# pmgbergen/porepy

Measured on NVIDIA H100. Metric: 3D cells/sec MPFA+MPSA assembly, higher is better.
Workload: dtype f64

## Files before the change

porepy_b200/csrc/mpsa_node.cuh:

```cuda
#pragma once
#include "node_kernels.cuh"

namespace pb {

PB_HD int mpsa_width(int nd, int nsf, int nsc, int nb, int nalpha) {
    return (nsf * nd + nsc * nd + nb * nd + nalpha * nsc) | 1;
}
PB_HD int64_t mpsa_A_doubles(int nd, int nsf, int nsc, int nb, int nalpha) {
    return (int64_t)nsf * nd * mpsa_width(nd, nsf, nsc, nb, nalpha);
}
PB_HD int64_t mpsa_rest_doubles(int nd, int nsf, int nsc, int nb, int nalpha) {
    const int64_t nd2 = nd * nd, n = (int64_t)nsf * nd;
    const int64_t nrhs = (int64_t)nsc * nd + (int64_t)nb * nd + (int64_t)nalpha * nsc;
    int64_t d = (int64_t)nsc * nd2 * nd2;
    d += (int64_t)nsc * nd2;
    d += nd2 * (n + (int64_t)nsc * nd);
    d += nd2 * nrhs;
    d += nsf;
    d += (int64_t)nsf * nd;
    d += (int64_t)nsc;
    d += (int64_t)nalpha * nsc * nd2 * 2;
    int64_t ints = nsc + 4 * (int64_t)nsf + (int64_t)nsf * nd + n + (int64_t)nsc * nd + 2 * nd;
    return d + (ints + 1) / 2 + 2;
}
// ... 96 lines not shown
        for (int q = 0; q < nal; ++q) {
            const double *al = prm.alpha + (int64_t)q * prm.alpha_stride;
            double a2[ND][ND];
#pragma unroll
            for (int a = 0; a < ND; ++a)
#pragma unroll
                for (int b = 0; b < ND; ++b) a2[a][b] = al[(3 * a + b) * prm.alpha_cs + c * prm.alpha_es];
#pragma unroll
            for (int m = 0; m < ND; ++m) {
                const int u = slot[k * ND + m] >> 1;
#pragma unroll
                for (int i = 0; i < ND; ++i) {
                    double v = 0.0, w = 0.0;
#pragma unroll
                    for (int r = 0; r < ND; ++r) {
                        v += nrm[u * ND + r] * a2[r][i];
                        w += a2[i][r] * Ei[r][m];
                    }
                    NA[((q * nsc + k) * ND + m) * ND + i] = v;
                    AE[((q * nsc + k) * ND + i) * ND + m] = w;
                }
            }
        }
    }
    t.sync();
    for (int it = t.tid(); it < nsc * ND2; it += t.size()) {
        const int k = it / ND2, p = it - k * ND2;
        const int64_t c = cell[k];
        const int pi = p / ND, pr = p - pi * ND;
        const double *Crow = prm.stiff + (int64_t)c9<ND>(pi, pr) * 9 * prm.stiff_cs + c * prm.stiff_es;
#pragma unroll
        for (int a = 0; a < ND; ++a) {
            double cs[ND];
#pragma unroll
            for (int q = 0; q < ND; ++q)
                cs[q] = sym_mask<ND>(p, a * ND + q) ? Crow[(int64_t)c9<ND>(a, q) * prm.stiff_cs] : 0.0;
#pragma unroll
            for (int m = 0; m < ND; ++m) {
                double v = 0.0;
#pragma unroll
                for (int q = 0; q < ND; ++q) v += cs[q] * E[k * ND2 + q * ND + m];
                PS[((k * ND2 + p) * ND + a) * ND + m] = v;
            }
        }
    }
    for (int it = t.tid(); it < ND2 * ND * nsc; it += t.size()) {
        const int pa = it / nsc, k = it - pa * nsc;
        const int p = pa / ND, a = pa - p * ND;
        const int pi = p / ND, pr = p - pi * ND;
        double tot = 0.0;
        for (int j = 0; j < nsc; ++j) tot += volk[j];
        const double w = volk[k] / tot;
        const int64_t c = cell[k];
        const double *Crow = prm.stiff + (int64_t)c9<ND>(pi, pr) * 9 * prm.stiff_cs + c * prm.stiff_es;
        double ca[ND];
#pragma unroll
        for (int q = 0; q < ND; ++q)
            ca[q] = sym_mask<ND>(p, a * ND + q) ? 0.0 : w * Crow[(int64_t)c9<ND>(a, q) * prm.stiff_cs];
        double sum = 0.0;
#pragma unroll
        for (int m = 0; m < ND; ++m) {
            double v = 0.0;
#pragma unroll
            for (int q = 0; q < ND; ++q) v += ca[q] * E[k * ND2 + q * ND + m];
            team_add(SA + p * n + (slot[k * ND + m] >> 1) * ND + a, v);
            sum += v;
        }
        SAc[p * ncc + k * ND + a] = -sum;
    }
    for (int i = t.tid(); i < ND; i += t.size()) {
        int cn = 0, cr = 0;
        for (int u = 0; u < nsf; ++u) {
            cn += bcu[u * ND + i] == 2;
            cr += bcu[u * ND + i] == 3;
        }
        elim[i] = nsc < cn;
        elim[ND + i] = nsc < cr;
    }
    t.sync();

    for (int u = t.tid(); u < nsf; u += t.size()) {
        const int s1 = sides[u] & 0xFFFF, s2 = (sides[u] >> 16) & 0xFFFF;
        int pick = s1;
        if (s2 != 0xFFFF) {
            const double *nu = nrm + u * ND;
            double w1 = 0.0, w2 = 0.0;
            const double *p1 = PS + (s1 / ND) * ND2 * ND2, *p2 = PS + (s2 / ND) * ND2 * ND2;
            for (int i = 0; i < ND; ++i)
                for (int am = 0; am < ND2; ++am) {
                    double a1 = 0.0, a2 = 0.0;
#pragma unroll
                    for (int r = 0; r < ND; ++r) {
                        a1 += nu[r] * p1[(i * ND + r) * ND2 + am];
                        a2 += nu[r] * p2[(i * ND + r) * ND2 + am];
                    }
                    w1 += fabs(a1);
                    w2 += fabs(a2);
                }
            if (w2 < w1) pick = s2;
        }
        sidesel[u] = pick;
    }
    t.sync();

    auto row_of = [&](int x, double *row) {
        const int u = x / ND, i = x - u * ND;
        const int code = bcu[x];
        if (code == 1 && prm.basis == nullptr) {
            row[x] = 1.0;
            row[n + ncc + bloc[u] * ND + i] = 1.0;
            return;
        }
        const double *nu = nrm + u * ND;
        if (prm.basis != nullptr && bloc[u] >= 0) {
            const int64_t fb = face[u];
            double B[ND][ND];
#pragma unroll
            for (int a = 0; a < ND; ++a)
#pragma unroll
                for (int j = 0; j < ND; ++j) B[a][j] = prm.basis[(int64_t)(a * ND + j) * nf + fb];
            if (code == 1) {
#pragma unroll
                for (int j = 0; j < ND; ++j) row[u * ND + j] = B[i][j];
                row[n + ncc + bloc[u] * ND + i] = 1.0;
            } else {
                const int side = sides[u] & 0xFFFF;
                const int k = side / ND;
                const double sg = (slot[side] & 1) ? -1.0 : 1.0;
                for (int j = 0; j < ND; ++j) {
                    const double wgt = sg * B[i][j];
                    if (wgt == 0.0) continue;
                    const double *ps = PS + (k * ND2 + j * ND) * ND2;
#pragma unroll
                    for (int a = 0; a < ND; ++a) {
                        double csum = 0.0;
#pragma unroll
                        for (int m = 0; m < ND; ++m) {
                            double v = 0.0;
#pragma unroll
                            for (int r = 0; r < ND; ++r) v += nu[r] * ps[(r * ND + a) * ND + m];
                            v *= wgt;
                            row[(slot[k * ND + m] >> 1) * ND + a] += v;
                            csum += v;
                        }
                        row[n + k * ND + a] += csum;
                    }
                    for (int q = 0; q < nal; ++q)
                        row[n + ncc + nbc + q * nsc + k] += wgt * NA[((q * nsc + k) * ND + (side - k * ND)) * ND + j];
                    const int cj = bcu[u * ND + j];
                    if (!((cj == 2 && elim[j]) || (cj == 3 && elim[ND + j]))) {
                        for (int c = 0; c < n; ++c) {
                            double v = 0.0;
#pragma unroll
                            for (int r = 0; r < ND; ++r) v += nu[r] * SA[(j * ND + r) * n + c];
                            row[c] += wgt * v;
                        }
                        for (int c = 0; c < ncc; ++c) {
                            double v = 0.0;
#pragma unroll
                            for (int r = 0; r < ND; ++r) v += nu[r] * SAc[(j * ND + r) * ncc + c];
                            row[n + c] -= wgt * v;
                        }
                    }
                }
                row[n + ncc + bloc[u] * ND + i] = invmf[u];
                if (code == 3) {
                    const double as = G.farea[fb] * invmf[u];
#pragma unroll
                    for (int j = 0; j < ND; ++j) {
                        double wb = 0.0;
#pragma unroll
                        for (int kk = 0; kk < ND; ++kk)
                            wb += (prm.robw ? prm.robw[(int64_t)(i * ND + kk) * nf + fb] : (i == kk ? 1.0 : 0.0)) * B[kk][j];
                        row[u * ND + j] += as * wb;
                    }
                }
            }
            return;
        }
        for (int sd = 0; sd < 2; ++sd) {
            const int side = sd == 0 ? (sides[u] & 0xFFFF) : ((sides[u] >> 16) & 0xFFFF);
            if (side == 0xFFFF) continue;
            const int k = side / ND;
            const double sg = (slot[side] & 1) ? -1.0 : 1.0;
            const double *ps = PS + (k * ND2 + i * ND) * ND2;
#pragma unroll
            for (int a = 0; a < ND; ++a) {
                double csum = 0.0;
#pragma unroll
                for (int m = 0; m < ND; ++m) {
                    double v = 0.0;
#pragma unroll
                    for (int r = 0; r < ND; ++r) v += nu[r] * ps[(r * ND + a) * ND + m];
                    v *= sg;
                    row[(slot[k * ND + m] >> 1) * ND + a] += v;
                    csum += v;
                }
                row[n + k * ND + a] += csum;
            }
            for (int q = 0; q < nal; ++q)
                row[n + ncc + nbc + q * nsc + k] += sg * NA[((q * nsc + k) * ND + (side - k * ND)) * ND + i];
            if (code != 0) {
                const bool el = code == 2 ? elim[i] : elim[ND + i];
                if (!el) {
                    for (int c = 0; c < n; ++c) {
                        double v = 0.0;
#pragma unroll
                        for (int r = 0; r < ND; ++r) v += nu[r] * SA[(i * ND + r) * n + c];
                        row[c] += sg * v;
                    }
                    for (int c = 0; c < ncc; ++c) {
                        double v = 0.0;
#pragma unroll
                        for (int r = 0; r < ND; ++r) v += nu[r] * SAc[(i * ND + r) * ncc + c];
                        row[n + c] -= sg * v;
                    }
                }
            }
        }
        if (code == 2 || code == 3) row[n + ncc + bloc[u] * ND + i] = invmf[u];
        if (code == 3) {
            const int64_t f = face[u];
            const double as = G.farea[f] * invmf[u];
#pragma unroll
            for (int j = 0; j < ND; ++j) {
                const double w = prm.robw ? prm.robw[(int64_t)(i * ND + j) * nf + f] : (i == j ? 1.0 : 0.0);
                row[u * ND + j] += as * w;
            }
        }
    };

    const double *X;
    int ldx;
    if (!Solver::solve_rows(t, row_of, n, nrhs, pool, rowidx, scratch, X, ldx)) {
        if (t.tid() == 0) flag_singular(err, s);
        t.sync();
        return;
    }

#if defined(__CUDA_ARCH__)
    int pf_sc0 = 0, pf_nsc = 0, pf_sf0 = 0, pf_nsf = 0;
    int64_t pf_pos0 = 0;
    if (s_next >= 0) {
        pf_sc0 = P.node_sc_ptr[s_next];
        pf_nsc = P.node_sc_ptr[s_next + 1] - pf_sc0;
        pf_sf0 = P.node_sf_ptr[s_next];
        pf_nsf = P.node_sf_ptr[s_next + 1] - pf_sf0;
        pf_pos0 = P.posfc_ptr[s_next];
    }
#endif
#if defined(__CUDA_ARCH__)
    {
        const int l = t.lane();
        const int ntr = (ND2 + 15) / 16, ntc = (nrhs + 7) / 8;
        for (int tile = t.warp(); tile < ntr * ntc; tile += t.nwarps()) {
            const int tr = tile / ntc, tc = tile - tr * ntc;
            const int row0 = 16 * tr + (l >> 2), row1 = row0 + 8;
            const int colb = 8 * tc + (l >> 2);
            double acc0[2] = {0.0, 0.0}, acc1[2] = {0.0, 0.0};
            for (int k0 = 0; k0 < n; k0 += 4) {
                const int k = k0 + (l & 3);
                const double a0 = (row0 < ND2 && k < n) ? SA[row0 * n + k] : 0.0;
                const double a1 = (row1 < ND2 && k < n) ? SA[row1 * n + k] : 0.0;
                const double b = (k < n && colb < nrhs) ? X[rowidx[k] * ldx + colb] : 0.0;
                pb_dmma2(acc0, acc1, a0, a1, b);
            }
            const int c0 = 8 * tc + 2 * (l & 3);
            const int rows[2] = {row0, row1};
            const double *accs[2] = {acc0, acc1};
            for (int h = 0; h < 2; ++h) {
                const int row = rows[h];
                if (row < ND2) {
                    if (c0 < nrhs) Z[row * nrhs + c0] = accs[h][0] + (c0 < ncc ? SAc[row * ncc + c0] : 0.0);
                    if (c0 + 1 < nrhs)
                        Z[row * nrhs + c0 + 1] = accs[h][1] + (c0 + 1 < ncc ? SAc[row * ncc + c0 + 1] : 0.0);
                }
            }
        }
    }
#else
    for (int it = t.tid(); it < ND2 * nrhs; it += t.size()) {
        const int p = it / nrhs, c = it - p * nrhs;
        double v = (c < ncc) ? SAc[p * ncc + c] : 0.0;
        for (int x = 0; x < n; ++x) v += SA[p * n + x] * X[(int64_t)rowidx[x] * ldx + c];
        Z[it] = v;
    }
#endif
    t.sync();

#if defined(__CUDA_ARCH__)
    int pf_cell = -1, pf_face = -1;
    if (t.tid() < pf_nsc) pf_cell = P.sc_cell[pf_sc0 + t.tid()];
    if (t.tid() < pf_nsf) {
        pf_face = P.sf_face[pf_sf0 + t.tid()];
        if ((t.tid() & 7) == 0) {
            pb_prefetch_l2(P.sf_sides + pf_sf0 + t.tid());
            pb_prefetch_l2(P.sf_bloc + pf_sf0 + t.tid());
        }
    }
    if (t.tid() * 16 < pf_nsc * ND) pb_prefetch_l2(P.slot_sf + (int64_t)pf_sc0 * ND + t.tid() * 16);
    for (int64_t off = (int64_t)t.tid() * 32; off < (int64_t)pf_nsf * pf_nsc; off += (int64_t)t.size() * 32)
        pb_prefetch_l2(P.pos_fc + pf_pos0 + off);
#endif
    const int32_t *pfc = P.pos_fc + P.posfc_ptr[s];
    const int32_t *pfb = P.pos_fb + P.posfb_ptr[s];
    for (int u = t.warp(); u < nsf; u += t.nwarps()) {
        const double *nu = nrm + u * ND;
        const int side1 = sidesel[u];
        const int k1 = side1 / ND, m1 = side1 - k1 * ND;
        double hs[ND][ND][ND];
        double hsum[ND][ND];
#pragma unroll
        for (int i = 0; i < ND; ++i) {
            const double *ps1 = PS + (k1 * ND2 + i * ND) * ND2;
#pragma unroll
            for (int a = 0; a < ND; ++a) {
                double sm = 0.0;
#pragma unroll
                for (int m = 0; m < ND; ++m) {
                    double v = 0.0;
#pragma unroll
                    for (int r = 0; r < ND; ++r) v += nu[r] * ps1[(r * ND + a) * ND + m];
                    hs[i][a][m] = v;
                    sm += v;
                }
                hsum[i][a] = sm;
            }
        }
        int xo[ND][ND];
#pragma unroll
        for (int a = 0; a < ND; ++a)
#pragma unroll
            for (int m = 0; m < ND; ++m) xo[a][m] = rowidx[(slot[k1 * ND + m] >> 1) * ND + a] * ldx;
        bool use_asym[ND];
        int uo[ND];
#pragma unroll
        for (int i = 0; i < ND; ++i) {
            const int code = bcu[u * ND + i];
            use_asym[i] = !((code == 2 && elim[i]) || (code == 3 && elim[ND + i]));
            uo[i] = rowidx[u * ND + i] * ldx;
        }
        const double im = invmf[u];
        const int64_t f = face[u];
        const int64_t fc0 = P.fc_indptr[f], fcl = P.fc_indptr[f + 1] - fc0;
        const int64_t fb0 = P.fb_indptr[f], fbl = P.fb_indptr[f + 1] - fb0;
        for (int c = t.lane(); c < nrhs; c += t.lanes()) {
            double hk[ND], tr[ND];
#pragma unroll
            for (int i = 0; i < ND; ++i) hk[i] = 0.0;
#pragma unroll
            for (int a = 0; a < ND; ++a)
#pragma unroll
                for (int m = 0; m < ND; ++m) {
                    const double xv = X[xo[a][m] + c];
#pragma unroll
                    for (int i = 0; i < ND; ++i) hk[i] += hs[i][a][m] * xv;
                }
#pragma unroll
            for (int i = 0; i < ND; ++i) {
                if (use_asym[i]) {
#pragma unroll
                    for (int r = 0; r < ND; ++r) hk[i] += nu[r] * Z[(i * ND + r) * nrhs + c];
                }
                tr[i] = X[uo[i] + c] * im;
            }
            if (c < ncc) {
                const int k = c / ND, j = c - k * ND;
                if (k == k1) {
#pragma unroll
                    for (int i = 0; i < ND; ++i) {
                        double hj = hsum[i][0];
#pragma unroll
                        for (int a = 1; a < ND; ++a) hj = (j == a) ? hsum[i][a] : hj;
                        hk[i] -= hj;
                    }
                }
                const int64_t pb = pfc[u * nsc + k];
                const int64_t pos = ND2 * fc0 + (pb - fc0) * ND + j;
#pragma unroll
                for (int i = 0; i < ND; ++i) {
                    if (o.stress) red_add(o.stress + pos + (int64_t)i * ND * fcl, hk[i]);
                    if (o.bdc) red_add(o.bdc + pos + (int64_t)i * ND * fcl, tr[i]);
                }
            } else if (c < ncc + nbc) {
                const int cb = c - ncc;
                const int b = cb / ND, j = cb - b * ND;
                const int64_t pb = pfb[u * nb + b];
                const int64_t pos = ND2 * fb0 + (pb - fb0) * ND + j;
#pragma unroll
                for (int i = 0; i < ND; ++i) {
                    if (o.bstress) red_add(o.bstress + pos + (int64_t)i * ND * fbl, hk[i]);
                    if (o.bdf) red_add(o.bdf + pos + (int64_t)i * ND * fbl, tr[i]);
                }
            } else {
                const int cq = c - ncc - nbc;
                const int q = cq / nsc, k = cq - q * nsc;
                const int64_t pb = pfc[u * nsc + k];
                const int64_t pos = ND * fc0 + (pb - fc0);
#pragma unroll
                for (int i = 0; i < ND; ++i) {
                    double h = hk[i];
                    if (k == k1) h -= NA[((q * nsc + k1) * ND + m1) * ND + i];
                    if (o.sg[q]) red_add(o.sg[q] + pos + (int64_t)i * fcl, h);
                    if (o.bdp[q]) red_add(o.bdp[q] + pos + (int64_t)i * fcl, tr[i]);
                }
            }
        }
    }
#if defined(__CUDA_ARCH__)
    if (pf_cell >= 0) {
        if (prm.stiff_cs == 1) {
            const double *rec = prm.stiff + (int64_t)pf_cell * prm.stiff_es;
#pragma unroll
            for (int b = 0; b < 81; b += 16) pb_prefetch_l2(rec + b);
            pb_prefetch_l2(rec + 80);
        }
        if (G.cell_cs == 1) pb_prefetch_l2(G.ccent + (int64_t)pf_cell * G.cell_es);
        pb_prefetch_l2(G.cvol + pf_cell);
        pb_prefetch_l2(P.sc_ncn + pf_cell);
    }
    if (pf_face >= 0) {
        if (G.face_cs == 1) {
            pb_prefetch_l2(G.fnorm + (int64_t)pf_face * G.face_es);
            pb_prefetch_l2(G.fcent + (int64_t)pf_face * G.face_es);
        }
        pb_prefetch_l2(P.fn_indptr + pf_face);
        pb_prefetch_l2(P.fc_indptr + pf_face);
#pragma unroll
        for (int i = 0; i < ND; ++i) pb_prefetch_l2(prm.bc + (int64_t)i * nf + pf_face);
    }
#endif
    if (nal > 0) {
        const int32_t *pcc = P.pos_cc + P.poscc_ptr[s];
        const int32_t *pcb = P.pos_cb + P.poscb_ptr[s];
        for (int it = t.warp(); it < nal * nsc; it += t.nwarps()) {
            const int q = it / nsc, k = it - q * nsc;
            const double *ae = AE + (q * nsc + k) * ND2;
            const double vol = volk[k];
            const double *xr[ND][ND];
#pragma unroll
            for (int a = 0; a < ND; ++a)
#pragma unroll
                for (int m = 0; m < ND; ++m)
                    xr[a][m] = X + (int64_t)rowidx[(slot[k * ND + m] >> 1) * ND + a] * ldx;
            for (int c = t.lane(); c < nrhs; c += t.lanes()) {
                double v = 0.0;
#pragma unroll
                for (int a = 0; a < ND; ++a)
#pragma unroll
                    for (int m = 0; m < ND; ++m) v += ae[a * ND + m] * xr[a][m][c];
                if (c < ncc) {
                    const int k2 = c / ND, j = c - k2 * ND;
                    if (k2 == k) {
#pragma unroll
                        for (int m = 0; m < ND; ++m) v -= ae[j * ND + m];
                    }
                    if (o.dd[q]) red_add(o.dd[q] + (int64_t)pcc[k * nsc + k2] * ND + j, vol * v);
                } else if (c < ncc + nbc) {
                    const int cb = c - ncc;
                    const int b = cb / ND, j = cb - b * ND;
                    if (o.bdd[q]) red_add(o.bdd[q] + (int64_t)pcb[k * nb + b] * ND + j, vol * v);
                } else {
                    const int cq = c - ncc - nbc;
                    const int q2 = cq / nsc, k2 = cq - q2 * nsc;
                    if (q2 == q && o.cons[q]) red_add(o.cons[q] + (int64_t)pcc[k * nsc + k2], vol * v);
                }
            }
        }
    }
    t.sync();
}

}
```

porepy_b200/csrc/node_kernels.cuh:

```cuda
#pragma once
#include <cmath>
#include <cstdint>

#include "views.hpp"

namespace pb {

struct CpuTeam {
    PB_HD int tid() const { return 0; }
    PB_HD int size() const { return 1; }
    PB_HD int lanes() const { return 1; }
    PB_HD int warp() const { return 0; }
    PB_HD int nwarps() const { return 1; }
    PB_HD int lane() const { return 0; }
    PB_HD void sync() const {}
    PB_HD void warp_argmax(double &, int &) const {}
};

#if defined(__CUDACC__)
template <int TEAM>
struct GpuTeam {
    __device__ __forceinline__ int tid() const { return TEAM == 32 ? (threadIdx.x & 31) : threadIdx.x; }
    __device__ __forceinline__ int size() const { return TEAM; }
    __device__ __forceinline__ int lanes() const { return 32; }
// ... 391 lines not shown
        double *Ainv = R + 4 * WP;
        int *prs = (int *)(Ainv + 16 * (NW + 1));
        int *usedf = prs + 8;
        for (int i = t.tid(); i < NP; i += t.size()) usedf[i] = i < n ? 0 : 1;
        for (int i = t.tid(); i < NP * 4; i += t.size()) P0[i] = 0.0;
        if (t.tid() == 0) prs[4] = 0;
        t.sync();
        const int npanel = (n + 3) >> 2;
        bool ok = true;
#pragma unroll
        for (int tcp = 0; tcp < NRT && tcp < NCT; ++tcp) {
            for (int half = 0; half < 2; ++half) {
                const int q = 2 * tcp + half;
                if (q >= npanel || !ok) break;
                const int p0 = 4 * q;
                const int pw = (n - p0) < 4 ? (n - p0) : 4;
                if (((l & 3) >> 1) == half) {
                    const int j0 = 2 * (l & 1);
#pragma unroll
                    for (int rt = 0; rt < RT; ++rt) {
                        const int myrow = 8 * (ti + NW * rt) + gr;
                        P0[myrow * 4 + j0] = c[rt][tcp][0];
                        P0[myrow * 4 + j0 + 1] = c[rt][tcp][1];
                    }
                }
                int myp[RT];
#pragma unroll
                for (int rt = 0; rt < RT; ++rt) {
                    const int myrow = 8 * (ti + NW * rt) + gr;
                    const int j = myrow - p0;
                    myp[rt] = (j >= 0 && j < pw) ? j : -1;
                    if (myp[rt] >= 0) {
#pragma unroll
                        for (int tc = tcp; tc < NCT; ++tc) {
                            Raw[myp[rt] * WP + 8 * tc + gc] = c[rt][tc][0];
                            Raw[myp[rt] * WP + 8 * tc + gc + 1] = c[rt][tc][1];
                        }
                    }
                }
                t.sync();
                double iv;
                const bool fast = try_diagonal_block(l, P0, usedf, p0, pw, iv);
                const double *ainv = Ainv;
                if (fast) {
                    double *mine = Ainv + 16 * (ti + 1);
                    if (l < 16) mine[l] = iv;
                    __syncwarp();
                    ainv = mine;
                } else {
                    t.sync();
                    if (ti == 0) factor_panel<false>(l, P0, usedf, prs, Ainv, rowidx, p0, pw);
                    t.sync();
                    ok = prs[4] == 0;
                    if (!ok) break;
#pragma unroll
                    for (int rt = 0; rt < RT; ++rt) {
                        const int myrow = 8 * (ti + NW * rt) + gr;
                        myp[rt] = -1;
#pragma unroll
                        for (int j = 0; j < 4; ++j)
                            if (prs[j] == myrow) myp[rt] = j;
                        if (myp[rt] >= 0) {
#pragma unroll
                            for (int tc = tcp; tc < NCT; ++tc) {
                                Raw[myp[rt] * WP + 8 * tc + gc] = c[rt][tc][0];
                                Raw[myp[rt] * WP + 8 * tc + gc + 1] = c[rt][tc][1];
                            }
                        }
                    }
                    t.sync();
                }
                for (int col = 8 * tcp + t.tid(); col < NCT * 8; col += t.size()) {
                    double raw[4];
#pragma unroll
                    for (int i = 0; i < 4; ++i) raw[i] = (i < pw) ? Raw[i * WP + col] : 0.0;
#pragma unroll
                    for (int j = 0; j < 4; ++j) {
                        double x = 0.0;
#pragma unroll
                        for (int i = 0; i < 4; ++i) x += ainv[j * 4 + i] * raw[i];
                        R[j * WP + col] = (j < pw) ? x : 0.0;
                    }
                }
                t.sync();
                if (fast && t.tid() < pw) {
                    usedf[p0 + t.tid()] = 1;
                    rowidx[p0 + t.tid()] = p0 + t.tid();
                }
                {
                    const int k = l & 3;
                    const int src = (l & ~3) | (2 * half + (k >> 1));
                    double af[RT];
#pragma unroll
                    for (int rt = 0; rt < RT; ++rt) {
                        const double v0 = __shfl_sync(0xffffffffu, c[rt][tcp][0], src);
                        const double v1 = __shfl_sync(0xffffffffu, c[rt][tcp][1], src);
                        af[rt] = (k < pw) ? -((k & 1) ? v1 : v0) : 0.0;
                    }
                    const double *rb = R + k * WP + (l >> 2);
#pragma unroll
                    for (int tc = tcp; tc < NCT; ++tc) {
                        const double bf = rb[8 * tc];
#pragma unroll
                        for (int rt = 0; rt + 1 < RT; rt += 2) pb_dmma2(c[rt][tc], c[rt + 1][tc], af[rt], af[rt + 1], bf);
                        if (RT & 1) pb_dmma(c[RT - 1][tc], af[RT - 1], bf);
                    }
#pragma unroll
                    for (int rt = 0; rt < RT; ++rt)
                        if (myp[rt] >= 0) {
#pragma unroll
                            for (int tc = tcp; tc < NCT; ++tc) {
                                c[rt][tc][0] = R[myp[rt] * WP + 8 * tc + gc];
                                c[rt][tc][1] = R[myp[rt] * WP + 8 * tc + gc + 1];
                            }
                        }
                }
            }
        }
        t.sync();
        return ok;
    }
};
#endif

#if defined(__CUDACC__)
__device__ __forceinline__ void pb_prefetch_l2(const void *p) {
    asm volatile("prefetch.global.L2 [%0];" ::"l"(p));
}
#endif

template <int ND>
PB_HD bool invert_small(const double (&D)[ND][ND], double (&E)[ND][ND]);

template <>
PB_HD bool invert_small<2>(const double (&D)[2][2], double (&E)[2][2]) {
    double det = D[0][0] * D[1][1] - D[0][1] * D[1][0];
    if (det == 0.0 || !(det == det)) return false;
    double id = 1.0 / det;
    E[0][0] = D[1][1] * id; E[0][1] = -D[0][1] * id;
    E[1][0] = -D[1][0] * id; E[1][1] = D[0][0] * id;
    return true;
}

template <>
PB_HD bool invert_small<3>(const double (&D)[3][3], double (&E)[3][3]) {
    double c00 = D[1][1] * D[2][2] - D[1][2] * D[2][1];
    double c01 = D[1][2] * D[2][0] - D[1][0] * D[2][2];
    double c02 = D[1][0] * D[2][1] - D[1][1] * D[2][0];
    double det = D[0][0] * c00 + D[0][1] * c01 + D[0][2] * c02;
    if (det == 0.0 || !(det == det)) return false;
    double id = 1.0 / det;
    E[0][0] = c00 * id;
    E[1][0] = c01 * id;
    E[2][0] = c02 * id;
    E[0][1] = (D[0][2] * D[2][1] - D[0][1] * D[2][2]) * id;
    E[1][1] = (D[0][0] * D[2][2] - D[0][2] * D[2][0]) * id;
    E[2][1] = (D[0][1] * D[2][0] - D[0][0] * D[2][1]) * id;
    E[0][2] = (D[0][1] * D[1][2] - D[0][2] * D[1][1]) * id;
    E[1][2] = (D[0][2] * D[1][0] - D[0][0] * D[1][2]) * id;
    E[2][2] = (D[0][0] * D[1][1] - D[0][1] * D[1][0]) * id;
    return true;
}

PB_HD int mpfa_width(int nd, int nsf, int nsc, int nb) { return (nsf + nsc + nb + nd * nsc) | 1; }
PB_HD int64_t mpfa_A_doubles(int nd, int nsf, int nsc, int nb) {
    return (int64_t)nsf * mpfa_width(nd, nsf, nsc, nb);
}
PB_HD int64_t mpfa_rest_doubles(int nd, int nsf, int nsc, int nb) {
    (void)nb;
    int64_t d = 2 * (int64_t)nsc * nd * nd + 2 * (int64_t)nsf;
    int64_t ints = nsc + 5 * (int64_t)nsf + (int64_t)nsc * nd;
    return d + (ints + 1) / 2 + 2;
}

template <int ND, class Solver, class Team>
PB_HD void mpfa_node(Team &t, const PlanView &P, const GeoView &G, const MpfaParams &prm,
                     const MpfaOut &o, int64_t s, double *A, double *smd, double *scratch, int *err) {
    const int sc0 = P.node_sc_ptr[s], nsc = P.node_sc_ptr[s + 1] - sc0;
    const int sf0 = P.node_sf_ptr[s], nsf = P.node_sf_ptr[s + 1] - sf0;
    const int nb = P.node_nb[s];
    if (nsf == 0) return;
    const int nrhs = nsc + nb + ND * nsc;
    const int W = (nsf + nrhs) | 1;
    const int64_t nf = P.nf, nc = P.nc, nn = P.nn;
    double *Tk = smd;
    double *Rk = Tk + nsc * ND * ND;
    double *invmf = Rk + nsc * ND * ND;
    double *robw = invmf + nsf;
    int *cell = (int *)(robw + nsf);
    int *face = cell + nsc;
    int *sides = face + nsf;
    int *bloc = sides + nsf;
    int *bcu = bloc + nsf;
    int *rowidx = bcu + nsf;
    int *slot = rowidx + nsf;

    for (int k = t.tid(); k < nsc; k += t.size()) cell[k] = P.sc_cell[sc0 + k];
    for (int i = t.tid(); i < nsc * ND; i += t.size()) slot[i] = P.slot_sf[(int64_t)sc0 * ND + i];
    for (int u = t.tid(); u < nsf; u += t.size()) {
        const int f = P.sf_face[sf0 + u];
        face[u] = f;
        sides[u] = (int)P.sf_sides[sf0 + u];
        const int bl = P.sf_bloc[sf0 + u];
        bloc[u] = (bl == 0xFFFF) ? -1 : bl;
        const double im = 1.0 / (double)(P.fn_indptr[f + 1] - P.fn_indptr[f]);
        invmf[u] = im;
        int code = 0;
        if (bl != 0xFFFF) {
            code = prm.bc[f];
            if (code == 0) code = 2;
        }
        bcu[u] = code;
        robw[u] = (code == 3 && prm.robw) ? prm.robw[f] * G.farea[f] * im : 0.0;
        rowidx[u] = u;
    }
    for (int i = t.tid(); i < nsf * W; i += t.size()) A[i] = 0.0;
    t.sync();

    for (int k = t.tid(); k < nsc; k += t.size()) {
        const int64_t c = cell[k];
        double xc[ND], xs[ND], K[ND][ND], D[ND][ND], R[ND][ND], E[ND][ND];
#pragma unroll
        for (int i = 0; i < ND; ++i) {
            xc[i] = G.ccent[i * G.cell_cs + c * G.cell_es];
            xs[i] = G.nodes[i * G.node_cs + s * G.node_es];
#pragma unroll
            for (int j = 0; j < ND; ++j) K[i][j] = prm.perm[(i * 3 + j) * prm.perm_cs + c * prm.perm_es];
        }
#pragma unroll
        for (int m = 0; m < ND; ++m) {
            const int u = slot[k * ND + m] >> 1;
            const int64_t f = face[u];
            const double e = (bloc[u] >= 0) ? 0.0 : prm.eta;
            double nrm[ND];
#pragma unroll
            for (int i = 0; i < ND; ++i) {
                const double xf = G.fcent[i * G.face_cs + f * G.face_es];
                D[m][i] = xf + e * (xs[i] - xf) - xc[i];
                nrm[i] = G.fnorm[i * G.face_cs + f * G.face_es] * invmf[u];
            }
#pragma unroll
            for (int j = 0; j < ND; ++j) {
                double a = 0.0;
#pragma unroll
                for (int i = 0; i < ND; ++i) a += nrm[i] * K[i][j];
                R[m][j] = a;
            }
        }
        if (!invert_small<ND>(D, E)) flag_singular(err, s);
#pragma unroll
        for (int m = 0; m < ND; ++m)
#pragma unroll
            for (int m2 = 0; m2 < ND; ++m2) {
                double a = 0.0;
#pragma unroll
                for (int q = 0; q < ND; ++q) a += R[m][q] * E[q][m2];
                Tk[k * ND * ND + m * ND + m2] = a;
                Rk[k * ND * ND + m * ND + m2] = R[m][m2];
            }
    }
    t.sync();

    for (int u = t.tid(); u < nsf; u += t.size()) {
        double *row = A + (int64_t)u * W;
        const int code = bcu[u];
        if (code == 1) {
            row[u] = 1.0;
            row[nsf + nsc + bloc[u]] = 1.0;
            continue;
        }
        for (int sd = 0; sd < 2; ++sd) {
            const int side = sd == 0 ? (sides[u] & 0xFFFF) : ((sides[u] >> 16) & 0xFFFF);
            if (side == 0xFFFF) continue;
            const int k = side / ND, m = side - k * ND;
            const double sg = (slot[side] & 1) ? -1.0 : 1.0;
            double tau = 0.0;
#pragma unroll
            for (int m2 = 0; m2 < ND; ++m2) {
                const int u2 = slot[k * ND + m2] >> 1;
                const double tt = sg * Tk[k * ND * ND + m * ND + m2];
                row[u2] += tt;
                tau += tt;
            }
            row[nsf + k] += tau;
#pragma unroll
            for (int j = 0; j < ND; ++j) row[nsf + nsc + nb + k * ND + j] += sg * Rk[k * ND * ND + m * ND + j];
        }
        if (code == 2 || code == 3) row[nsf + nsc + bloc[u]] = -invmf[u];
        if (code == 3) row[u] -= robw[u];
        double sum = 0.0;
        for (int c = 0; c < nsf; ++c) sum += fabs(row[c]);
        if (!(sum > 0.0)) { flag_singular(err, s); continue; }
        const double is = 1.0 / sum;
        for (int c = 0; c < nsf + nrhs; ++c) row[c] *= is;
    }
    t.sync();

    if (!Solver::solve(t, A, nsf, W, nrhs, rowidx, scratch)) {
        if (t.tid() == 0) flag_singular(err, s);
        t.sync();
        return;
    }

    const int32_t *pfc = P.pos_fc + P.posfc_ptr[s];
    const int32_t *pfb = P.pos_fb + P.posfb_ptr[s];
    for (int u = t.warp(); u < nsf; u += t.nwarps()) {
        int side1 = sides[u] & 0xFFFF;
        {
            const int side2 = (sides[u] >> 16) & 0xFFFF;
            if (side2 != 0xFFFF) {
                double n1 = 0.0, n2 = 0.0;
#pragma unroll
                for (int m2 = 0; m2 < ND; ++m2) {
                    n1 += fabs(Tk[side1 * ND + m2]);
                    n2 += fabs(Tk[side2 * ND + m2]);
                }
                if (n2 < n1) side1 = side2;
            }
        }
        const int k1 = side1 / ND, m1 = side1 - k1 * ND;
        const double *T1 = Tk + k1 * ND * ND + m1 * ND;
        const double *R1 = Rk + k1 * ND * ND + m1 * ND;
        const double *xrow[ND];
        double tau1 = 0.0;
#pragma unroll
        for (int m2 = 0; m2 < ND; ++m2) {
            xrow[m2] = A + (int64_t)rowidx[slot[k1 * ND + m2] >> 1] * W + nsf;
            tau1 += T1[m2];
        }
        const double *xu = A + (int64_t)rowidx[u] * W + nsf;
        const double im = invmf[u];
        for (int c = t.lane(); c < nrhs; c += t.lanes()) {
            double fl = 0.0;
#pragma unroll
            for (int m2 = 0; m2 < ND; ++m2) fl -= T1[m2] * xrow[m2][c];
            const double tr = xu[c] * im;
            if (c < nsc) {
                if (c == k1) fl += tau1;
                const int64_t p = pfc[u * nsc + c];
                if (o.flux) red_add(o.flux + p, fl);
                if (o.bpc) red_add(o.bpc + p, tr);
            } else if (c < nsc + nb) {
                const int64_t p = pfb[u * nb + (c - nsc)];
                if (o.bflux) red_add(o.bflux + p, fl);
                if (o.bpf) red_add(o.bpf + p, tr);
            } else {
                const int cc = c - nsc - nb;
                const int k = cc / ND, j = cc - k * ND;
                if (k == k1) fl += R1[j];
                const int64_t p = (int64_t)pfc[u * nsc + k] * ND + j;
                if (o.vs) red_add(o.vs + p, fl);
                if (o.bpvs) red_add(o.bpvs + p, tr);
            }
        }
    }
    t.sync();
}

}
```

Before: 7.325 million.

## Flatten scatter loops over (face,rhs) pairs with shared precomputed tables

Both the MPFA and MPSA scatter phases now distribute flattened (subface, rhs column) pairs across all team threads instead of assigning one subface per warp with lanes striding columns. Per-subface data (stress hs tensors, row offsets, asymmetry mask, face index ranges, position tables) is precomputed once into scratch buffers (reused A/SA/PS/E regions) after a sync. The aim is better thread utilization when nrhs is small relative to the warp width, and less redundant per-lane computation. It adds extra syncs and relies on scratch regions being large enough and no longer needed, and it introduces per-thread division and shared-memory indirection.

```diff
diff --git a/porepy_b200/csrc/mpsa_node.cuh b/porepy_b200/csrc/mpsa_node.cuh
--- a/porepy_b200/csrc/mpsa_node.cuh
+++ b/porepy_b200/csrc/mpsa_node.cuh
@@ -422,108 +422,123 @@
     for (int64_t off = (int64_t)t.tid() * 32; off < (int64_t)pf_nsf * pf_nsc; off += (int64_t)t.size() * 32)
         pb_prefetch_l2(P.pos_fc + pf_pos0 + off);
 #endif
+    constexpr int ND3 = ND2 * ND, XW = ND2 + ND + 1;
+    double *hs = SA;
     const int32_t *pfc = P.pos_fc + P.posfc_ptr[s];
+    const bool stage = nsf <= 2 * ND3;
+    const int32_t *pfs = stage ? (const int32_t *)SAc : pfc;
+    int *frow = (int *)E;
+    int *xo = (int *)PS;
+    for (int it = t.tid(); it < nsf * ND3; it += t.size()) {
+        const int u = it / ND3, iam = it - u * ND3;
+        const int i = iam / ND2, am = iam - i * ND2;
+        const double *nu = nrm + u * ND;
+        const double *ps1 = PS + ((sidesel[u] / ND) * ND2 + i * ND) * ND2 + am;
+        double v = 0.0;
+#pragma unroll
+        for (int r = 0; r < ND; ++r) v += nu[r] * ps1[r * ND2];
+        hs[it] = v;
+    }
+    if (stage)
+        for (int it = t.tid(); it < nsf * nsc; it += t.size()) ((int32_t *)SAc)[it] = pfc[it];
+    for (int u = t.tid(); u < nsf; u += t.size()) {
+        const int64_t f = face[u];
+        const int fc0 = P.fc_indptr[f];
+        frow[4 * u] = fc0;
+        frow[4 * u + 1] = P.fc_indptr[f + 1] - fc0;
+        const int fb0 = nb > 0 ? P.fb_indptr[f] : 0;
+        frow[4 * u + 2] = fb0;
+        frow[4 * u + 3] = nb > 0 ? P.fb_indptr[f + 1] - fb0 : 0;
+    }
+    t.sync();
+    for (int u = t.tid(); u < nsf; u += t.size()) {
+        const int k1 = sidesel[u] / ND;
+        int *xu = xo + u * XW;
+#pragma unroll
+        for (int m = 0; m < ND; ++m) {
+            const int x0 = (slot[k1 * ND + m] >> 1) * ND;
+#pragma unroll
+            for (int a = 0; a < ND; ++a) xu[a * ND + m] = rowidx[x0 + a] * ldx;
+        }
+        int v = 0;
+#pragma unroll
+        for (int i = 0; i < ND; ++i) {
+            const int code = bcu[u * ND + i];
+            if (!((code == 2 && elim[i]) || (code == 3 && elim[ND + i]))) v |= 1 << i;
+        }
+        xu[ND2 + ND] = v;
+#pragma unroll
+        for (int i = 0; i < ND; ++i) xu[ND2 + i] = rowidx[u * ND + i] * ldx;
+    }
+    t.sync();
     const int32_t *pfb = P.pos_fb + P.posfb_ptr[s];
-    for (int u = t.warp(); u < nsf; u += t.nwarps()) {
+    for (int it = t.tid(); it < nsf * nrhs; it += t.size()) {
+        const int u = it / nrhs, c = it - u * nrhs;
         const double *nu = nrm + u * ND;
+        const double *hu = hs + u * ND3;
+        const int *xu = xo + u * XW;
         const int side1 = sidesel[u];
         const int k1 = side1 / ND, m1 = side1 - k1 * ND;
-        double hs[ND][ND][ND];
-        double hsum[ND][ND];
+        double hk[ND], tr[ND];
+#pragma unroll
+        for (int i = 0; i < ND; ++i) hk[i] = 0.0;
+#pragma unroll
+        for (int a = 0; a < ND; ++a)
+#pragma unroll
+            for (int m = 0; m < ND; ++m) {
+                const double xv = X[xu[a * ND + m] + c];
+#pragma unroll
+                for (int i = 0; i < ND; ++i) hk[i] += hu[(i * ND + a) * ND + m] * xv;
+            }
+        const int asym = xu[ND2 + ND];
+        const double im = invmf[u];
 #pragma unroll
         for (int i = 0; i < ND; ++i) {
-            const double *ps1 = PS + (k1 * ND2 + i * ND) * ND2;
-#pragma unroll
-            for (int a = 0; a < ND; ++a) {
-                double sm = 0.0;
-#pragma unroll
-                for (int m = 0; m < ND; ++m) {
-                    double v = 0.0;
-#pragma unroll
-                    for (int r = 0; r < ND; ++r) v += nu[r] * ps1[(r * ND + a) * ND + m];
-                    hs[i][a][m] = v;
-                    sm += v;
-                }
-                hsum[i][a] = sm;
-            }
-        }
-        int xo[ND][ND];
-#pragma unroll
-        for (int a = 0; a < ND; ++a)
-#pragma unroll
-            for (int m = 0; m < ND; ++m) xo[a][m] = rowidx[(slot[k1 * ND + m] >> 1) * ND + a] * ldx;
-        bool use_asym[ND];
-        int uo[ND];
-#pragma unroll
-        for (int i = 0; i < ND; ++i) {
-            const int code = bcu[u * ND + i];
-            use_asym[i] = !((code == 2 && elim[i]) || (code == 3 && elim[ND + i]));
-            uo[i] = rowidx[u * ND + i] * ldx;
-        }
-        const double im = invmf[u];
-        const int64_t f = face[u];
-        const int64_t fc0 = P.fc_indptr[f], fcl = P.fc_indptr[f + 1] - fc0;
-        const int64_t fb0 = P.fb_indptr[f], fbl = P.fb_indptr[f + 1] - fb0;
-        for (int c = t.lane(); c < nrhs; c += t.lanes()) {
-            double hk[ND], tr[ND];
-#pragma unroll
-            for (int i = 0; i < ND; ++i) hk[i] = 0.0;
-#pragma unroll
-            for (int a = 0; a < ND; ++a)
-#pragma unroll
-                for (int m = 0; m < ND; ++m) {
-                    const double xv = X[xo[a][m] + c];
-#pragma unroll
-                    for (int i = 0; i < ND; ++i) hk[i] += hs[i][a][m] * xv;
-                }
+            if ((asym >> i) & 1) {
+#pragma unroll
+                for (int r = 0; r < ND; ++r) hk[i] += nu[r] * Z[(i * ND + r) * nrhs + c];
+            }
+            tr[i] = X[xu[ND2 + i] + c] * im;
+        }
+        if (c < ncc) {
+            const int k = c / ND, j = c - k * ND;
+            if (k == k1) {
+#pragma unroll
+                for (int i = 0; i < ND; ++i) {
+                    double hj = 0.0;
+#pragma unroll
+                    for (int m = 0; m < ND; ++m) hj += hu[(i * ND + j) * ND + m];
+                    hk[i] -= hj;
+                }
+            }
+            const int64_t fc0 = frow[4 * u], fcl = frow[4 * u + 1];
+            const int64_t pos = ND2 * fc0 + (pfs[u * nsc + k] - fc0) * ND + j;
 #pragma unroll
             for (int i = 0; i < ND; ++i) {
-                if (use_asym[i]) {
-#pragma unroll
-                    for (int r = 0; r < ND; ++r) hk[i] += nu[r] * Z[(i * ND + r) * nrhs + c];
-                }
-                tr[i] = X[uo[i] + c] * im;
-            }
-            if (c < ncc) {
-                const int k = c / ND, j = c - k * ND;
-                if (k == k1) {
-#pragma unroll
-                    for (int i = 0; i < ND; ++i) {
-                        double hj = hsum[i][0];
-#pragma unroll
-                        for (int a = 1; a < ND; ++a) hj = (j == a) ? hsum[i][a] : hj;
-                        hk[i] -= hj;
-                    }
-                }
-                const int64_t pb = pfc[u * nsc + k];
-                const int64_t pos = ND2 * fc0 + (pb - fc0) * ND + j;
-#pragma unroll
-                for (int i = 0; i < ND; ++i) {
-                    if (o.stress) red_add(o.stress + pos + (int64_t)i * ND * fcl, hk[i]);
-                    if (o.bdc) red_add(o.bdc + pos + (int64_t)i * ND * fcl, tr[i]);
-                }
-            } else if (c < ncc + nbc) {
-                const int cb = c - ncc;
-                const int b = cb / ND, j = cb - b * ND;
-                const int64_t pb = pfb[u * nb + b];
-                const int64_t pos = ND2 * fb0 + (pb - fb0) * ND + j;
-#pragma unroll
-                for (int i = 0; i < ND; ++i) {
-                    if (o.bstress) red_add(o.bstress + pos + (int64_t)i * ND * fbl, hk[i]);
-                    if (o.bdf) red_add(o.bdf + pos + (int64_t)i * ND * fbl, tr[i]);
-                }
-            } else {
-                const int cq = c - ncc - nbc;
-                const int q = cq / nsc, k = cq - q * nsc;
-                const int64_t pb = pfc[u * nsc + k];
-                const int64_t pos = ND * fc0 + (pb - fc0);
-#pragma unroll
-                for (int i = 0; i < ND; ++i) {
-                    double h = hk[i];
-                    if (k == k1) h -= NA[((q * nsc + k1) * ND + m1) * ND + i];
-                    if (o.sg[q]) red_add(o.sg[q] + pos + (int64_t)i * fcl, h);
-                    if (o.bdp[q]) red_add(o.bdp[q] + pos + (int64_t)i * fcl, tr[i]);
-                }
+                if (o.stress) red_add(o.stress + pos + (int64_t)i * ND * fcl, hk[i]);
+                if (o.bdc) red_add(o.bdc + pos + (int64_t)i * ND * fcl, tr[i]);
+            }
+        } else if (c < ncc + nbc) {
+            const int cb = c - ncc;
+            const int b = cb / ND, j = cb - b * ND;
+            const int64_t fb0 = frow[4 * u + 2], fbl = frow[4 * u + 3];
+            const int64_t pos = ND2 * fb0 + (pfb[u * nb + b] - fb0) * ND + j;
+#pragma unroll
+            for (int i = 0; i < ND; ++i) {
+                if (o.bstress) red_add(o.bstress + pos + (int64_t)i * ND * fbl, hk[i]);
+                if (o.bdf) red_add(o.bdf + pos + (int64_t)i * ND * fbl, tr[i]);
+            }
+        } else {
+            const int cq = c - ncc - nbc;
+            const int q = cq / nsc, k = cq - q * nsc;
+            const int64_t fc0 = frow[4 * u], fcl = frow[4 * u + 1];
+            const int64_t pos = ND * fc0 + (pfs[u * nsc + k] - fc0);
+#pragma unroll
+            for (int i = 0; i < ND; ++i) {
+                double h = hk[i];
+                if (k == k1) h -= NA[((q * nsc + k1) * ND + m1) * ND + i];
+                if (o.sg[q]) red_add(o.sg[q] + pos + (int64_t)i * fcl, h);
+                if (o.bdp[q]) red_add(o.bdp[q] + pos + (int64_t)i * fcl, tr[i]);
             }
         }
     }
diff --git a/porepy_b200/csrc/node_kernels.cuh b/porepy_b200/csrc/node_kernels.cuh
--- a/porepy_b200/csrc/node_kernels.cuh
+++ b/porepy_b200/csrc/node_kernels.cuh
@@ -717,9 +717,8 @@
         return;
     }
 
-    const int32_t *pfc = P.pos_fc + P.posfc_ptr[s];
-    const int32_t *pfb = P.pos_fb + P.posfb_ptr[s];
-    for (int u = t.warp(); u < nsf; u += t.nwarps()) {
+    int *sel = bcu;
+    for (int u = t.tid(); u < nsf; u += t.size()) {
         int side1 = sides[u] & 0xFFFF;
         {
             const int side2 = (sides[u] >> 16) & 0xFFFF;
@@ -733,43 +732,55 @@
                 if (n2 < n1) side1 = side2;
             }
         }
-        const int k1 = side1 / ND, m1 = side1 - k1 * ND;
-        const double *T1 = Tk + k1 * ND * ND + m1 * ND;
-        const double *R1 = Rk + k1 * ND * ND + m1 * ND;
-        const double *xrow[ND];
-        double tau1 = 0.0;
-#pragma unroll
-        for (int m2 = 0; m2 < ND; ++m2) {
-            xrow[m2] = A + (int64_t)rowidx[slot[k1 * ND + m2] >> 1] * W + nsf;
-            tau1 += T1[m2];
-        }
-        const double *xu = A + (int64_t)rowidx[u] * W + nsf;
-        const double im = invmf[u];
-        for (int c = t.lane(); c < nrhs; c += t.lanes()) {
-            double fl = 0.0;
-#pragma unroll
-            for (int m2 = 0; m2 < ND; ++m2) fl -= T1[m2] * xrow[m2][c];
-            const double tr = xu[c] * im;
-            if (c < nsc) {
-                if (c == k1) fl += tau1;
-                const int64_t p = pfc[u * nsc + c];
-                if (o.flux) red_add(o.flux + p, fl);
-                if (o.bpc) red_add(o.bpc + p, tr);
-            } else if (c < nsc + nb) {
-                const int64_t p = pfb[u * nb + (c - nsc)];
-                if (o.bflux) red_add(o.bflux + p, fl);
-                if (o.bpf) red_add(o.bpf + p, tr);
-            } else {
-                const int cc = c - nsc - nb;
-                const int k = cc / ND, j = cc - k * ND;
-                if (k == k1) fl += R1[j];
-                const int64_t p = (int64_t)pfc[u * nsc + k] * ND + j;
-                if (o.vs) red_add(o.vs + p, fl);
-                if (o.bpvs) red_add(o.bpvs + p, tr);
-            }
+        sel[u] = side1;
+        int *xo = (int *)(A + (int64_t)u * W) + nsc;
+        const int k1 = side1 / ND;
+#pragma unroll
+        for (int m2 = 0; m2 < ND; ++m2) xo[m2] = rowidx[slot[k1 * ND + m2] >> 1] * W;
+    }
+    {
+        const int32_t *pfc = P.pos_fc + P.posfc_ptr[s];
+        for (int it = t.tid(); it < nsf * nsc; it += t.size()) {
+            const int u = it / nsc, k = it - u * nsc;
+            ((int *)(A + (int64_t)u * W))[k] = pfc[it];
         }
     }
     t.sync();
-}
-
-}
+    const int32_t *pfb = P.pos_fb + P.posfb_ptr[s];
+    for (int it = t.tid(); it < nsf * nrhs; it += t.size()) {
+        const int u = it / nrhs, c = it - u * nrhs;
+        const int side1 = sel[u];
+        const int k1 = side1 / ND;
+        const double *T1 = Tk + side1 * ND;
+        const int *pfs = (const int *)(A + (int64_t)u * W), *xo = pfs + nsc;
+        double fl = 0.0;
+#pragma unroll
+        for (int m2 = 0; m2 < ND; ++m2) fl -= T1[m2] * A[xo[m2] + nsf + c];
+        const double tr = A[(int64_t)rowidx[u] * W + nsf + c] * invmf[u];
+        if (c < nsc) {
+            if (c == k1) {
+                double tau1 = 0.0;
+#pragma unroll
+                for (int m2 = 0; m2 < ND; ++m2) tau1 += T1[m2];
+                fl += tau1;
+            }
+            const int64_t p = pfs[c];
+            if (o.flux) red_add(o.flux + p, fl);
+            if (o.bpc) red_add(o.bpc + p, tr);
+        } else if (c < nsc + nb) {
+            const int64_t p = pfb[u * nb + (c - nsc)];
+            if (o.bflux) red_add(o.bflux + p, fl);
+            if (o.bpf) red_add(o.bpf + p, tr);
+        } else {
+            const int cc = c - nsc - nb;
+            const int k = cc / ND, j = cc - k * ND;
+            if (k == k1) fl += Rk[side1 * ND + j];
+            const int64_t p = (int64_t)pfs[k] * ND + j;
+            if (o.vs) red_add(o.vs + p, fl);
+            if (o.bpvs) red_add(o.bpvs + p, tr);
+        }
+    }
+    t.sync();
+}
+
+}
```

Result: faster. 7.640 million (median of 6 runs) (+4.3%).
